# leggedrobotics/delora

Hardware: AMD Instinct MI355X
Metric: training scan-pairs/sec, KITTI 64x2048 range images (higher is better)
Workload: dtype f32; 1 GPU; KITTI-shaped 64x2048, batch=8 pairs/GPU, raw scans of ~141k points (ragged, raster order), steps rotate over 8 distinct HBM-resident batches, online normals, ResNet pose CNN (11.9M params, identity-pretrained state), Adam; BASELINE configs[1]; global_batch=8, parallelism=dp1, cnn=fp32, cnn_impl=hip trunk: fp32 MFMA, fused Winograd F(2x2,3x3) + direct implicit GEMM, channels_last=False, hip_graph=False, distinct_batches=8, priming_steps=8

## Files before the change

delora_amd/_lib.py:

```python
import ctypes
import os

_HERE = os.path.dirname(os.path.abspath(__file__))
LIB_PATH = os.path.join(_HERE, "csrc", "libdelora_hip.so")
ABI_VERSION = 10


class DeloraHipError(RuntimeError):
    pass


class SensorStruct(ctypes.Structure):
    _fields_ = [("H", ctypes.c_int32), ("W", ctypes.c_int32),
                ("hfov0", ctypes.c_double), ("hfov1", ctypes.c_double),
                ("vfov0", ctypes.c_double), ("vfov1", ctypes.c_double)]


_vp, _i32, _i64, _u32, _f32, _sz = (ctypes.c_void_p, ctypes.c_int32, ctypes.c_int64, ctypes.c_uint32,
                                    ctypes.c_float, ctypes.c_size_t)
_SP = ctypes.POINTER(SensorStruct)

SIGNATURES = {
    "dl_abi_version": (_i32, []),
    "dl_last_error": (ctypes.c_char_p, []),
    "dl_project_workspace_bytes": (_sz, [_i32, _i32, _i32, _i64, _i32]),
    "dl_project": (_i32, [_vp, _i64, _i64, _vp, _i32, _i32, _i32, _SP, _vp, _vp, _vp, _vp, _vp, _vp, _vp, _vp, _vp]),
    "dl_reproject_workspace_bytes": (_sz, [_i32, _i32, _i32]),
    "dl_reproject": (_i32, [_vp, _i64, _vp, _i64, _vp, _i64, _vp, _vp, _i32, _SP, _vp, _vp, _vp, _vp, _vp]),
    "dl_normals": (_i32, [_vp, _i64, _i32, _i32, _i32, _i32, _i32, _f32, _i32, _vp, _vp, _vp]),
    "dl_nn_workspace_bytes": (_sz, [_i32, _i32, _i32]),
    "dl_nn_correspond": (_i32, [_vp, _i64, _vp, _i64, _vp, _i64, _vp, _i64, _vp, _i32, _SP, _i32, _vp, _vp, _vp, _vp, _vp]),
    "dl_icp_loss_workspace_bytes": (_sz, [_i32, _i32, _i32]),
    "dl_icp_loss_fwd": (_i32, [_vp, _i64, _vp, _i64, _vp, _i64, _vp, _vp, _i32, _i32, _i32, _u32,
                               _vp, _vp, _vp, _vp, _vp]),
    "dl_icp_loss_partial": (_i32, [_vp, _i64, _vp, _i64, _vp, _i64, _vp, _vp, _i32, _i32, _i32, _u32, _vp, _vp]),
    "dl_icp_loss_reduce": (_i32, [_vp, _i32, _i32, _i32, _u32, _vp, _vp, _vp, _vp]),
    "dl_icp_loss_bwd": (_i32, [_vp, _vp, _i32, _vp, _vp]),
    "dl_ring_act_pool_pad_fwd": (_i32, [_vp, _i64, _i32, _i32, _i32, _vp, _vp, _vp]),
    "dl_ring_act_pool_pad_bwd": (_i32, [_vp, _vp, _vp, _i64, _i32, _i32, _i32, _vp, _vp]),
    "dl_timer_create": (_i32, [ctypes.POINTER(ctypes.c_void_p)]),
    "dl_timer_destroy": (_i32, [_vp]),
    "dl_timer_elapsed_ms": (_i32, [_vp, ctypes.POINTER(ctypes.c_float)]),
    "dl_icp_loss_partial_timed": (_i32, [_vp, _i64, _vp, _i64, _vp, _i64, _vp, _vp, _i32, _i32, _i32, _u32, _vp, _vp, _vp]),
    "dl_probe_stream_read": (_i32, [_vp, _i64, _vp, _i64, _vp, _i64, _vp, _i32, _i32, _i32, _vp, _vp]),
    "dl_nn_bruteforce": (_i32, [_vp, _i64, _i32, _vp, _i64, _i32, _vp, _vp]),
    "dl_nn_list_tree_bytes": (_sz, [_i32]),
    "dl_nn_list_query_workspace_bytes": (_sz, [_i32]),
    "dl_nn_list_build": (_i32, [_vp, _i64, _i32, _vp, _vp]),
    "dl_nn_list_query": (_i32, [_vp, _i64, _i32, _vp, _i64, _i32, _vp, _vp, _vp, _vp]),
    "dl_ring_act_pad_fwd": (_i32, [_vp, _vp, _i64, _i64, _i64, _i32, _i32, _i32, _vp, _vp]),
    "dl_ring_act_pad_bwd": (_i32, [_vp, _vp, _i64, _i32, _i32, _i32, _vp, _vp, _vp]),
    "dl_ring_act_pad_fwd_t": (_i32, [_vp, _vp, _i64, _i64, _i64, _i32, _i32, _i32, _i32, _vp, _vp]),
    "dl_ring_act_pad_bwd_t": (_i32, [_vp, _vp, _i64, _i32, _i32, _i32, _i32, _vp, _vp, _vp]),
    "dl_ring_act_pool_pad_fwd_t": (_i32, [_vp, _i64, _i32, _i32, _i32, _i32, _vp, _vp, _vp]),
    "dl_ring_act_pool_pad_bwd_t": (_i32, [_vp, _vp, _vp, _i64, _i32, _i32, _i32, _i32, _vp, _vp]),
    "dl_conv2d_nhwc_f32": (_i32, [_vp, _vp, _vp, _vp, _vp, _i32, _i32, _i32, _i32, _i32, _i32, _i32, _i32, _i32, _i32, _u32, _vp]),
    "dl_conv2d_dgrad_strided_nhwc_f32": (_i32, [_vp, _vp, _vp, _vp, _vp, _i32, _i32, _i32, _i32, _i32, _i32, _i32, _i32, _i32, _i32,
                                                _u32, _vp, _vp]),
    "dl_conv2d_wgrad_workspace_bytes": (_sz, [_i32, _i32, _i32, _i32, _i32, _i32, _i32, _i32]),
    "dl_conv2d_wgrad_nhwc_f32": (_i32, [_vp, _vp, _vp, _vp, _i32, _i32, _i32, _i32, _i32, _i32, _i32, _i32, _vp]),
    "dl_tower_conv3x3_nhwc_f32": (_i32, [_vp, _vp, _vp, _vp, _i32, _i32, _i32, _i32, _i32, _vp, _vp, _vp, _i32, _i32, _u32, _vp]),
    "dl_tower_wgrad_workspace_bytes": (_sz, [_i32, _i32, _i32, _i32, _i32]),
    "dl_tower_wgrad3x3_nhwc_f32": (_i32, [_vp, _vp, _vp, _vp, _i32, _i32, _i32, _i32, _i32, _vp, _vp, _vp]),
    "dl_wino_weights_floats": (_sz, [_i32, _i32]),
    "dl_wino_weights_f32": (_i32, [_vp, _vp, _vp, _i32, _i32, _vp]),
    "dl_wino_weights_batch_f32": (_i32, [_vp, _i32, _vp]),
    "dl_wino_conv3x3_workspace_bytes": (_sz, [_i32, _i32, _i32, _i32, _i32]),
    "dl_wino_conv3x3_nhwc_f32": (_i32, [_vp, _vp, _vp, _vp, _vp, _i32, _i32, _i32, _i32, _i32, _i32, _u32, _vp, _vp]),
    "dl_wino_wgrad_workspace_bytes": (_sz, [_i32, _i32, _i32, _i32, _i32]),
    "dl_wino_wgrad3x3_nhwc_f32": (_i32, [_vp, _vp, _vp, _vp, _i32, _i32, _i32, _i32, _i32, _vp]),
    "dl_pool3x3s12_nhwc_fwd": (_i32, [_vp, _i32, _i32, _i32, _i32, _vp, _vp, _vp]),
    "dl_pool3x3s12_nhwc_bwd": (_i32, [_vp, _vp, _vp, _i32, _i32, _i32, _i32, _i32, _vp, _vp]),
    "dl_stem_wgrad_workspace_bytes": (_sz, [_i32, _i32, _i32]),
    "dl_stem_wgrad_f32": (_i32, [_vp, _vp, _vp, _vp, _i32, _i32, _i32, _i32, _vp, _vp, _vp]),
    "dl_quat_to_T_fwd": (_i32, [_vp, _vp, _i32, ctypes.c_float, _vp, _vp]),
    "dl_quat_to_T_bwd": (_i32, [_vp, _vp, _i32, ctypes.c_float, _vp, _vp, _vp]),
    "dl_mean_hw_nhwc_f32": (_i32, [_vp, _i32, _i32, _i32, _vp, _vp]),
    "dl_conv_weights_h": (_i32, [_vp, _vp, _vp, _i32, _i32, _i32, _i32, _vp]),
    "dl_conv_weights_batch_h": (_i32, [_vp, _i32, _i32, _vp]),
    "dl_conv2d_nhwc_h": (_i32, [_vp, _vp, _vp, _vp, _vp, _i32, _i32, _i32, _i32, _i32, _i32, _i32, _i32, _i32, _i32, _i32, _u32, _vp]),
    "dl_conv2d_dgrad_strided_nhwc_h": (_i32, [_vp, _vp, _vp, _vp, _vp, _i32, _i32, _i32, _i32, _i32, _i32, _i32, _i32, _i32, _i32, _i32,
                                              _u32, _vp, _vp]),
    "dl_cast_f32_to_h": (_i32, [_vp, _vp, _i64, _i32, _vp]),
    "dl_heads_fwd": (_i32, [_vp, _vp, _i32, _i32, _i32, _i32, _i32, _vp, _vp, _vp, _vp, _vp, _vp, _vp]),
    "dl_heads_bwd_workspace_bytes": (_sz, [_i32, _i32, _i32, _i32]),
    "dl_heads_bwd": (_i32, [_vp, _vp, _i32, _i32, _i32, _i32, _i32, _vp, _vp, _vp, _vp, _vp, _vp, _vp, _vp, _vp, _vp]),
    "dl_heads_fwd_drop": (_i32, [_vp, _vp, _i32, _i32, _i32, _i32, _i32, _vp, _vp, _vp, _vp, _vp, _vp, _vp, _vp]),
    "dl_heads_bwd_drop": (_i32, [_vp, _vp, _i32, _i32, _i32, _i32, _i32, _vp, _vp, _vp, _vp, _vp, _vp, _vp, _vp, _vp, _vp, _vp]),
    "dl_heads_single_fwd": (_i32, [_vp, _vp, _i32, _i32, _i32, _i32, _i32, _i32, _i32, _i32, _vp, _vp, _vp, _vp, _vp, _vp, _vp]),
# ... 120 lines not shown
```

delora_amd/csrc/conv.hip:

```cpp
#include <type_traits>

#include "common.h"
#include "conv_geom.h"

typedef float f32x16 __attribute__((ext_vector_type(16)));
typedef float f32x4 __attribute__((ext_vector_type(4)));

__device__ __forceinline__ __amdgpu_buffer_rsrc_t cv_rsrc(const float* base, unsigned bytes) {
  return __builtin_amdgcn_make_buffer_rsrc(const_cast<float*>(base), 0, (int)bytes, 0x00020000);
}
__device__ __forceinline__ f32x4 cv_ld16(__amdgpu_buffer_rsrc_t rs, unsigned voff, unsigned soff) {
  return __builtin_bit_cast(f32x4, __builtin_amdgcn_raw_buffer_load_b128(rs, (int)voff, (int)soff, 0));
}
#define CV_ZERO_OFF 0x80000000u

#define CV_THREADS 256
#define CV_EPI_ADD 1u
#define CV_EPI_ACT 2u
#define CV_EPI_DACT 4u
#define CV_EPI_ADD_GRID 8u
#define CV_ACT_NONE 0
#define CV_ACT_TANH 1
#define CV_ACT_RELU 2

struct ConvArgs {
  const float* x;
  const float* w;
  float* y;
  const float* add;
  const float* dsrc;
  int N, H, W, C, K, Ho, Wo;
  int act;
  unsigned epi;
  int Hout, Wout;
  int wrap;
  const float* seam;
};

__device__ __forceinline__ float cv_act(float v, int act) {
  if (act == CV_ACT_TANH) return dl_tanh(v);
  if (act == CV_ACT_RELU) return v < 0.f ? 0.f : v;
  return v;
}
__device__ __forceinline__ float cv_dact(float y, int act) {
  if (act == CV_ACT_TANH) return 1.f - y * y;
  if (act == CV_ACT_RELU) return y <= 0.f ? 0.f : 1.f;
  return 1.f;
}

__device__ __forceinline__ int cv_xcd_swizzle(int id, int n) {
  const int q = n / 8, r = n % 8, xcd = id % 8, k = id / 8;
  return (xcd < r ? xcd * (q + 1) : r * (q + 1) + (xcd - r) * q) + k;
}

template <int BM, int BN, int CK, int TW, class G, bool BT, int WGN>
#ifndef CV_MINWAVES
#define CV_MINWAVES 2
#endif
__global__ __launch_bounds__(CV_THREADS, CV_MINWAVES) void k_conv_f32(ConvArgs a) {
  constexpr int TH = BM / TW;
  constexpr int SH = G::ISH, SW = G::ISW;
  constexpr int RH = (TH - 1) * SH + G::EH, RW = (TW - 1) * SW + G::EW;
  constexpr int S = CK + 4;
  constexpr int TAPS = G::NT;
  constexpr int C4 = CK / 4;
  constexpr int IN_FLOATS = RH * RW * S;
  constexpr int W_FLOATS = BT ? TAPS * CK * BN : TAPS * BN * S;
  constexpr int NI = RH * RW * C4;
  constexpr int NW = BT ? CK * TAPS * (BN / 4) : BN * TAPS * C4;
  constexpr int NI_IT = (NI + CV_THREADS - 1) / CV_THREADS, NW_IT = (NW + CV_THREADS - 1) / CV_THREADS;
  constexpr int WGM = 4 / WGN;
  constexpr int WM = BM / 32 / WGM, WN = BN / 32 / WGN;
  static_assert(BM % TW == 0 && BM % (32 * WGM) == 0 && BN % (32 * WGN) == 0 && CK % 8 == 0, "tile shape");
  static_assert(TAPS > 0, "a stride phase without taps has no launch");
  static_assert((S / 4) % 2 == 1, "pixel stride must be 4*odd floats");
  constexpr int EPW = WN * 32, ES = EPW + 4;
  constexpr int LDS_HOLD = (BM == 256 && TW == 128 && CK == 8 && BT) ? 160 * 1024 / 3 / 4 + 16 : 0;
  constexpr int LDS_USED = IN_FLOATS + W_FLOATS > 4 * 32 * ES ? IN_FLOATS + W_FLOATS : 4 * 32 * ES;
  constexpr int LDS_FLOATS = LDS_USED > LDS_HOLD ? LDS_USED : LDS_HOLD;
  __shared__ __attribute__((aligned(16))) float lds[LDS_FLOATS];
  float* in_lds = lds;
  float* w_lds = lds + IN_FLOATS;

  const int tid = threadIdx.x, lane = tid & 63, wave = tid >> 6;
  const int li = lane & 31, half = lane >> 5;
  const int wm = wave / WGN, wn = wave % WGN;
  const int KT = a.K / BN;
  const int tiles_w = (a.Wo + TW - 1) / TW, tiles_h = (a.Ho + TH - 1) / TH;
  const int ntiles = a.N * tiles_h * tiles_w * KT;
  const int t = cv_xcd_swizzle(blockIdx.x, ntiles);
  const int kt = t % KT;
  int pt = t / KT;
  const int tw_i = pt % tiles_w; pt /= tiles_w;
  const int th_i = pt % tiles_h;
  const int n = pt / tiles_h;
  const int ho0 = th_i * TH, wo0 = tw_i * TW, k0 = kt * BN;
  const int h_base = ho0 * SH + G::H0, w_base = wo0 * SW + G::W0;
  const float* xn = a.x + (size_t)n * a.H * a.W * a.C;

  const unsigned x_bytes = (unsigned)(a.H * a.W * a.C) * 4u, w_bytes = (unsigned)(a.K * a.C * G::WTAPS) * 4u;
  const __amdgpu_buffer_rsrc_t x_rs = cv_rsrc(xn, x_bytes), w_rs = cv_rsrc(a.w, w_bytes);
  const unsigned x_zero = CV_ZERO_OFF;
  unsigned in_g[NI_IT];
  int in_l[NI_IT];
#pragma unroll
  for (int it = 0; it < NI_IT; ++it) {
    const int q = min(tid + it * CV_THREADS, NI - 1);
    const int c4 = q % C4, pc = q / C4;
    const int col = pc % RW, row = pc / RW;
    const int h = h_base + row;
    int w = w_base + col;
    const bool col_in = w >= 0 && w < a.W;
    w = w < 0 ? w + a.W : w;
    w = w >= a.W ? w - a.W : w;
    in_l[it] = pc * S + c4 * 4;
    in_g[it] = (h >= 0 && h < a.H && (a.wrap ? w < a.W : col_in)) ? (unsigned)((h * a.W + w) * a.C + c4 * 4) * 4u : x_zero;
  }
  unsigned w_g[NW_IT];
  int w_l[NW_IT];
#pragma unroll
  for (int it = 0; it < NW_IT; ++it) {
    const int q = min(tid + it * CV_THREADS, NW - 1);
    if (!BT) {
      const int c4 = q % C4, t2 = q / C4;
      const int tap = t2 % TAPS, kk = t2 / TAPS;
      w_g[it] = (unsigned)(((k0 + kk) * G::WTAPS + G::wt(tap)) * a.C + c4 * 4) * 4u;
      w_l[it] = (tap * BN + kk) * S + c4 * 4;
    } else {
      const int co4 = q % (BN / 4), t2 = q / (BN / 4);
      const int tap = t2 % TAPS, kr = t2 / TAPS;
      w_g[it] = (unsigned)((kr * G::WTAPS + G::wt(tap)) * a.K + k0 + co4 * 4) * 4u;
      w_l[it] = (tap * CK + kr) * BN + co4 * 4;
    }
  }

  f32x16 acc[WM][WN];
#pragma unroll
  for (int i = 0; i < WM; ++i)
#pragma unroll
    for (int j = 0; j < WN; ++j)
#pragma unroll
      for (int r = 0; r < 16; ++r) acc[i][j][r] = 0.f;

  int a_off[WM];
#pragma unroll
  for (int mi = 0; mi < WM; ++mi) {
    const int p = (wm * WM + mi) * 32 + li;
    const int th = p / TW, tw = p % TW;
    a_off[mi] = ((th * SH) * RW + tw * SW) * S + half * 4;
  }

  f32x4 in_r[NI_IT], w_r[NW_IT];
#define CV_FETCH(C0)                                                                                                      \
  {                                                                                                                       \
    const unsigned xs_ = (unsigned)(C0) * 4u, ws_ = BT ? (unsigned)((C0) * G::WTAPS * a.K) * 4u : xs_;          \
    _Pragma("unroll") for (int it = 0; it < NI_IT; ++it) in_r[it] = cv_ld16(x_rs, in_g[it], xs_);                         \
    _Pragma("unroll") for (int it = 0; it < NW_IT; ++it) w_r[it] = cv_ld16(w_rs, w_g[it], ws_);                           \
  }
#define CV_STAGE()                                                                                                        \
  {                                                                                                                       \
    _Pragma("unroll") for (int it = 0; it < NI_IT; ++it) *reinterpret_cast<f32x4*>(in_lds + in_l[it]) = in_r[it];         \
    _Pragma("unroll") for (int it = 0; it < NW_IT; ++it) *reinterpret_cast<f32x4*>(w_lds + w_l[it]) = w_r[it];            \
  }

  CV_FETCH(0)
  CV_STAGE()
  __syncthreads();
  for (int c0 = 0; c0 < a.C; c0 += CK) {
    const bool more = c0 + CK < a.C;
    if (more) CV_FETCH(c0 + CK)
#ifdef CV_OLD_LOOP
#pragma unroll
    for (int tap = 0; tap < TAPS; ++tap) {
#pragma unroll
      for (int kq = 0; kq < CK / 8; ++kq) {
        float4 af[WM];
#pragma unroll
        for (int mi = 0; mi < WM; ++mi)
          af[mi] = *reinterpret_cast<const float4*>(in_lds + a_off[mi] + (G::dh(tap) * RW + G::dw(tap)) * S + kq * 8);
        float bf[WN][4];
#pragma unroll
        for (int ni = 0; ni < WN; ++ni) {
          const int col = (wn * WN + ni) * 32 + li;
          if (!BT) {
            const float4 v = *reinterpret_cast<const float4*>(w_lds + (tap * BN + col) * S + kq * 8 + half * 4);
            bf[ni][0] = v.x; bf[ni][1] = v.y; bf[ni][2] = v.z; bf[ni][3] = v.w;
          } else {
#pragma unroll
            for (int j = 0; j < 4; ++j) bf[ni][j] = w_lds[(tap * CK + kq * 8 + half * 4 + j) * BN + col];
          }
        }
#pragma unroll
        for (int j = 0; j < 4; ++j)
#pragma unroll
          for (int mi = 0; mi < WM; ++mi) {
            const float av = j == 0 ? af[mi].x : (j == 1 ? af[mi].y : (j == 2 ? af[mi].z : af[mi].w));
#pragma unroll
            for (int ni = 0; ni < WN; ++ni)
              acc[mi][ni] = __builtin_amdgcn_mfma_f32_32x32x2f32(av, bf[ni][j], acc[mi][ni], 0, 0, 0);
          }
      }
    }
#else
    constexpr int KQ = CK / 8, NSTEP = TAPS * KQ;
    float4 af[2][WM];
    float bf[2][WN][4];
    auto load_frags = [&](int step, int buf) {
      const int tap = step / KQ, kq = step % KQ;
#pragma unroll
      for (int mi = 0; mi < WM; ++mi)
        af[buf][mi] = *reinterpret_cast<const float4*>(in_lds + a_off[mi] + (G::dh(tap) * RW + G::dw(tap)) * S + kq * 8);
#pragma unroll
      for (int ni = 0; ni < WN; ++ni) {
        const int col = (wn * WN + ni) * 32 + li;
        if (!BT) {
          const float4 v = *reinterpret_cast<const float4*>(w_lds + (tap * BN + col) * S + kq * 8 + half * 4);
          bf[buf][ni][0] = v.x; bf[buf][ni][1] = v.y; bf[buf][ni][2] = v.z; bf[buf][ni][3] = v.w;
        } else {
#pragma unroll
          for (int j = 0; j < 4; ++j) bf[buf][ni][j] = w_lds[(tap * CK + kq * 8 + half * 4 + j) * BN + col];
        }
      }
    };
    load_frags(0, 0);
#pragma unroll
    for (int step = 0; step < NSTEP; ++step) {
      const int cur = step & 1;
      if (step + 1 < NSTEP) load_frags(step + 1, cur ^ 1);
#pragma unroll
      for (int j = 0; j < 4; ++j)
#pragma unroll
        for (int mi = 0; mi < WM; ++mi) {
          const float av = j == 0 ? af[cur][mi].x : (j == 1 ? af[cur][mi].y : (j == 2 ? af[cur][mi].z : af[cur][mi].w));
#pragma unroll
          for (int ni = 0; ni < WN; ++ni)
            acc[mi][ni] = __builtin_amdgcn_mfma_f32_32x32x2f32(av, bf[cur][ni][j], acc[mi][ni], 0, 0, 0);
        }
#ifndef CV_NO_SGB
      if (step + 1 < NSTEP) __builtin_amdgcn_sched_group_barrier(0x100, WM + (BT ? 4 * WN : WN), 0);
      __builtin_amdgcn_sched_group_barrier(0x008, 4 * WM * WN, 0);
#endif
    }
#endif
    __syncthreads();
    if (more) {
      CV_STAGE()
      __syncthreads();
    }
  }

  __syncthreads();
  float* ep = lds + wave * (32 * ES);
  const unsigned out_n = (unsigned)(n * a.Hout * a.Wout), grid_n = (unsigned)(n * a.Ho * a.Wo);
  const unsigned k_lane = (unsigned)(k0 + wn * EPW);
  const bool f_add = a.epi & CV_EPI_ADD, f_act = a.epi & CV_EPI_ACT, f_dact = a.epi & CV_EPI_DACT;
  const bool f_addg = a.epi & CV_EPI_ADD_GRID;
#pragma unroll
  for (int mi = 0; mi < WM; ++mi) {
#pragma unroll
    for (int ni = 0; ni < WN; ++ni)
#pragma unroll
      for (int r = 0; r < 16; ++r) ep[((r & 3) + 8 * (r >> 2) + 4 * half) * ES + ni * 32 + li] = acc[mi][ni][r];
#pragma unroll 2
    for (int q = lane; q < 32 * (EPW / 4); q += 64) {
      const int row = q / (EPW / 4), c4 = q % (EPW / 4);
      const int p = (wm * WM + mi) * 32 + row;
      const int th = p / TW, tw = p % TW;
      const int oh = (ho0 + th) * G::OSH + G::OPH, ow = (wo0 + tw) * G::OSW + G::OPW;
      if (ho0 + th >= a.Ho || wo0 + tw >= a.Wo || oh >= a.Hout || ow >= a.Wout) continue;
      const unsigned o = (out_n + (unsigned)(oh * a.Wout + ow)) * (unsigned)a.K + k_lane + c4 * 4;
      float4 v = *reinterpret_cast<const float4*>(ep + row * ES + c4 * 4);
      if (a.seam && (ow == 0 || ow == a.Wout - 1)) {
        const float4 t = *reinterpret_cast<const float4*>(a.seam + ((unsigned)((n * a.Hout + oh) * 2 + (ow != 0)) * (unsigned)a.K + k_lane + c4 * 4));
        v.x += t.x; v.y += t.y; v.z += t.z; v.w += t.w;
      }
      if (f_addg) {
        const float4 t = *reinterpret_cast<const float4*>(a.add + ((grid_n + (unsigned)((ho0 + th) * a.Wo + (wo0 + tw))) * (unsigned)a.K + k_lane + c4 * 4));
        v.x += t.x; v.y += t.y; v.z += t.z; v.w += t.w;
      }
      if (f_add) {
        const float4 t = *reinterpret_cast<const float4*>(a.add + o);
        v.x += t.x; v.y += t.y; v.z += t.z; v.w += t.w;
      }
      if (f_act) { v.x = cv_act(v.x, a.act); v.y = cv_act(v.y, a.act); v.z = cv_act(v.z, a.act); v.w = cv_act(v.w, a.act); }
      if (f_dact) {
        const float4 t = *reinterpret_cast<const float4*>(a.dsrc + o);
        v.x *= cv_dact(t.x, a.act); v.y *= cv_dact(t.y, a.act); v.z *= cv_dact(t.z, a.act); v.w *= cv_dact(t.w, a.act);
      }
      *reinterpret_cast<float4*>(a.y + o) = v;
    }
  }
}

#undef CV_FETCH
#undef CV_STAGE

struct WgArgs {
  const float* x;
  const float* g;
  float* part;
  int N, H, W, C, K, Ho, Wo, chunks_per_slab, nslabs;
};
template <int BMK, int BNC, int PK, int SH, int SW, int KS, bool FAST>
__device__ __forceinline__ void wgrad_f32_body(const float* __restrict__ x, const float* __restrict__ g, float* __restrict__ part, int N, int H,
                                               int W, int C, int K, int Ho, int Wo, int chunks_per_slab, int nslabs, const int blk) {
  constexpr int PAD = (KS - 1) / 2;
  constexpr int TAPS = KS * KS;
  constexpr int RW = (PK - 1) * SW + KS;
  constexpr int X_FLOATS = KS * RW * BNC, G_FLOATS = PK * BMK;
  constexpr int NX = KS * RW * (BNC / 4), NG = PK * (BMK / 4);
  constexpr int NX_IT = (NX + CV_THREADS - 1) / CV_THREADS, NG_IT = (NG + CV_THREADS - 1) / CV_THREADS;
  constexpr int TM = BMK / 32, TN = BNC / 32;
  constexpr int TILES = TM * TN;
  static_assert(TILES % 4 == 0, "tile count");
  constexpr int TPW = TILES / 4;
  __shared__ __attribute__((aligned(16))) float lds[X_FLOATS + G_FLOATS];
  float* x_lds = lds;
  float* g_lds = lds + X_FLOATS;
  const int tid = threadIdx.x, lane = tid & 63, wave = tid >> 6;
  const int li = lane & 31, half = lane >> 5;
  const int KT = K / BMK, CT = C / BNC;
  int t = blk;
// ... 373 lines not shown
  }
}

extern "C" int dl_conv2d_nhwc_f32(const float* x, const float* w, float* y, const float* add, const float* dsrc, int32_t N,
                                  int32_t H, int32_t W, int32_t C, int32_t K, int32_t ksize, int32_t stride_h,
                                  int32_t stride_w, int32_t transposed, int32_t act, uint32_t epilogue, dl_stream stream) {
  if (!x || !w || !y || N <= 0 || H <= 0 || W <= 0 || C <= 0 || K <= 0)
    return dl_fail(DL_ERR_INVALID_ARGUMENT, "dl_conv2d_nhwc_f32: bad argument");
  if (((epilogue & CV_EPI_ADD) && !add) || ((epilogue & CV_EPI_DACT) && !dsrc) || act < 0 || act > 2 || (epilogue & ~7u))
    return dl_fail(DL_ERR_INVALID_ARGUMENT, "dl_conv2d_nhwc_f32: epilogue operand missing / bad activation or flag");
  if ((stride_h != 1 && stride_h != 2) || (stride_w != 1 && stride_w != 2) || (ksize != 1 && ksize != 3))
    return dl_fail(DL_ERR_INVALID_ARGUMENT, "dl_conv2d_nhwc_f32: kernel size must be 1 or 3, strides 1 or 2 (got %d, %d, %d)", ksize, stride_h, stride_w);
  if ((size_t)N * H * W * C >= ((size_t)1 << 31) || (size_t)N * H * W * K >= ((size_t)1 << 31))
    return dl_fail(DL_ERR_UNSUPPORTED, "dl_conv2d_nhwc_f32: tensors beyond 2^31 elements are not supported (split the batch)");
  if ((size_t)H * W * C >= ((size_t)1 << 29) || (size_t)K * C * ksize * ksize >= ((size_t)1 << 29))
    return dl_fail(DL_ERR_UNSUPPORTED, "dl_conv2d_nhwc_f32: an image or the weights of 2 GiB and more are not supported");
  const int Ho = (H + stride_h - 1) / stride_h, Wo = (W + stride_w - 1) / stride_w;
  ConvArgs a{x, w, y, add, dsrc, N, H, W, C, K, Ho, Wo, act, epilogue, Ho, Wo, 1, nullptr};
  hipStream_t st = (hipStream_t)stream;
  int rc = 1;
  if (ksize == 3 && stride_h == 1 && stride_w == 1)
    rc = transposed ? dispatch_conv<GeomDgrad<3, 1, 1, 0, 0, false>, true, true>(a, st) : dispatch_conv<GeomConv<3, 1, 1>, false, true>(a, st);
  else if (transposed) return dl_fail(DL_ERR_UNSUPPORTED, "dl_conv2d_nhwc_f32: transposed weights need stride 1, 3x3 (strided layers: dl_conv2d_dgrad_strided_nhwc_f32)");
  else if (ksize == 3 && stride_h == 1 && stride_w == 2) rc = dispatch_conv<GeomConv<3, 1, 2>, false, false>(a, st);
  else if (ksize == 3 && stride_h == 2 && stride_w == 2) rc = dispatch_conv<GeomConv<3, 2, 2>, false, false>(a, st);
  else if (ksize == 1 && stride_h == 1 && stride_w == 2) rc = dispatch_conv<GeomConv<1, 1, 2>, false, false>(a, st);
  else if (ksize == 1 && stride_h == 2 && stride_w == 2) rc = dispatch_conv<GeomConv<1, 2, 2>, false, false>(a, st);
  else return dl_fail(DL_ERR_UNSUPPORTED, "dl_conv2d_nhwc_f32: kernel %d stride (%d,%d) is not built", ksize, stride_h, stride_w);
  if (rc) return dl_fail(DL_ERR_UNSUPPORTED, "dl_conv2d_nhwc_f32: shape N=%d H=%d W=%d C=%d K=%d does not tile (K %% %d, C %% 8)",
                         N, H, W, C, K, CV_BN);
  return dl_check_launch("dl_conv2d_nhwc_f32");
}

template <int KS, int SH, int SW, int PH, int PW>
static int dgrad_phase(ConvArgs a, bool first_phase, hipStream_t st) {
  using G = GeomDgrad<KS, SH, SW, PH, PW, true>;
  if (!first_phase) a.epi &= ~CV_EPI_ADD_GRID;
  if constexpr (G::NT > 0) return dispatch_conv<G, true, false>(a, st);
  return 1;
}

extern "C" int dl_conv2d_dgrad_strided_nhwc_f32(const float* g, const float* w, float* dx, const float* add_grid, const float* dsrc,
                                                int32_t N, int32_t H, int32_t W, int32_t K, int32_t C, int32_t ksize,
                                                int32_t stride_h, int32_t stride_w, int32_t dense, int32_t act,
                                                uint32_t epilogue, float* seam_ws, dl_stream stream) {
  if (!g || !w || !dx || N <= 0 || H <= 0 || W <= 0 || C <= 0 || K <= 0)
    return dl_fail(DL_ERR_INVALID_ARGUMENT, "dl_conv2d_dgrad_strided_nhwc_f32: bad argument");
  if (((epilogue & CV_EPI_ADD_GRID) && !add_grid) || ((epilogue & CV_EPI_DACT) && !dsrc) || act < 0 || act > 2 ||
      (epilogue & ~(CV_EPI_ADD_GRID | CV_EPI_DACT)))
    return dl_fail(DL_ERR_INVALID_ARGUMENT, "dl_conv2d_dgrad_strided_nhwc_f32: epilogue operand missing / unsupported flag");
  if ((stride_h != 1 && stride_h != 2) || (stride_w != 1 && stride_w != 2) || (ksize != 1 && ksize != 3))
    return dl_fail(DL_ERR_INVALID_ARGUMENT, "dl_conv2d_dgrad_strided_nhwc_f32: kernel size must be 1 or 3, strides 1 or 2 (got %d, %d, %d)", ksize, stride_h, stride_w);
  const int Ho = (H + stride_h - 1) / stride_h, Wo = (W + stride_w - 1) / stride_w;
  if ((size_t)N * H * W * C >= ((size_t)1 << 31) || (size_t)N * Ho * Wo * K >= ((size_t)1 << 31))
    return dl_fail(DL_ERR_UNSUPPORTED, "dl_conv2d_dgrad_strided_nhwc_f32: tensors beyond 2^31 elements are not supported");
  if ((size_t)Ho * Wo * K >= ((size_t)1 << 29) || (size_t)K * C * ksize * ksize >= ((size_t)1 << 29))
    return dl_fail(DL_ERR_UNSUPPORTED, "dl_conv2d_dgrad_strided_nhwc_f32: an image or the weights of 2 GiB and more are not supported");
  const bool odd_w = stride_w == 2 && (W & 1) && ksize == 3 && !dense && W >= 3;
  if (odd_w && !seam_ws)
    return dl_fail(DL_ERR_INVALID_ARGUMENT, "dl_conv2d_dgrad_strided_nhwc_f32: an odd image width (%d) needs seam_ws (N*H*2*C floats)", W);
  ConvArgs a{g, w, dx, add_grid, dsrc, N, Ho, Wo, K, C, Ho, Wo, act, epilogue, dense ? Ho : H, dense ? Wo : W, odd_w ? 0 : 1,
             odd_w ? seam_ws : nullptr};
  hipStream_t st = (hipStream_t)stream;
  if (odd_w) {
    const int row_tiles = (H + FX_ROWS - 1) / FX_ROWS;
    DL_LAUNCH_PLAIN(k_dgrad_oddw_seam, dim3(N * row_tiles, 2, (C + 63) / 64), dim3(CV_THREADS), st, g, w, seam_ws, N, Ho, Wo, K, C, H, stride_h);
// ... 208 lines not shown
```

delora_amd/csrc/conv_geom.h:

```cpp
#pragma once

template <int KS_, int SH_, int SW_>
struct GeomConv {
  static constexpr int NT = KS_ * KS_, WTAPS = KS_ * KS_, ISH = SH_, ISW = SW_;
  static constexpr int H0 = -((KS_ - 1) / 2), W0 = -((KS_ - 1) / 2), EH = KS_, EW = KS_;
  static constexpr int OSH = 1, OSW = 1, OPH = 0, OPW = 0;
  static constexpr int dh(int t) { return t / KS_; }
  static constexpr int dw(int t) { return t % KS_; }
  static constexpr int wt(int t) { return t; }
};

template <int KS_, int S_, int P_>
struct DgradAxis {
  static constexpr int PAD = (KS_ - 1) / 2;
  static constexpr bool valid(int r) { return (P_ + PAD - r) % S_ == 0; }
  static constexpr int off(int r) { return (P_ + PAD - r) / S_; }
  static constexpr int count() { int n = 0; for (int r = 0; r < KS_; ++r) n += valid(r) ? 1 : 0; return n; }
  static constexpr int tap(int i) { int n = 0; for (int r = 0; r < KS_; ++r) if (valid(r)) { if (n == i) return r; ++n; } return 0; }
  static constexpr int lo() { int m = 99; for (int r = 0; r < KS_; ++r) if (valid(r) && off(r) < m) m = off(r); return m; }
  static constexpr int hi() { int m = -99; for (int r = 0; r < KS_; ++r) if (valid(r) && off(r) > m) m = off(r); return m; }
};

template <int KS_, int SH_, int SW_, int PH_, int PW_, bool SO_>
struct GeomDgrad {
  using AH = DgradAxis<KS_, SH_, PH_>;
  using AW = DgradAxis<KS_, SW_, PW_>;
  static constexpr int NR = AH::count(), NS = AW::count();
  static constexpr int NT = NR * NS, WTAPS = KS_ * KS_, ISH = 1, ISW = 1;
  static constexpr int H0 = AH::lo(), W0 = AW::lo(), EH = AH::hi() - AH::lo() + 1, EW = AW::hi() - AW::lo() + 1;
  static constexpr int OSH = SO_ ? SH_ : 1, OSW = SO_ ? SW_ : 1, OPH = SO_ ? PH_ : 0, OPW = SO_ ? PW_ : 0;
  static constexpr int dh(int t) { return AH::off(AH::tap(t / NS)) - H0; }
  static constexpr int dw(int t) { return AW::off(AW::tap(t % NS)) - W0; }
  static constexpr int wt(int t) { return AH::tap(t / NS) * KS_ + AW::tap(t % NS); }
};
```

delora_amd/models/ring_conv.py:

```python
import ctypes
import os

import torch

from .. import _lib

ACT = {"none": 0, "tanh": 1, "relu": 2}
USE_WINOGRAD = True
EPI_ADD, EPI_ACT, EPI_DACT, EPI_ADD_GRID = 1, 2, 4, 8


def _ptr(t):
    return ctypes.c_void_p(t.data_ptr()) if t is not None else ctypes.c_void_p(0)


def _stream():
    return ctypes.c_void_p(torch.cuda.current_stream().cuda_stream)


ALLOC_SKEW = 0
_skew_state = {"i": 0}


def _empty(shape, dtype, device):
# ... 4 lines not shown
        n *= int(d)
    esz = torch.empty((), dtype=dtype).element_size()
    _skew_state["i"] = (_skew_state["i"] + 1) % 8
    off = (_skew_state["i"] * ALLOC_SKEW) // esz
    return torch.empty((n + (8 * ALLOC_SKEW) // esz,), dtype=dtype, device=device)[off:off + n].view(shape)


def weight_storage(w):
    v = w.permute(0, 2, 3, 1)
    return v if v.is_contiguous() else v.contiguous()


def grad_for(dw_krsc, w_param):
    shape, stride = (tuple(w_param.shape), tuple(w_param.stride())) if torch.is_tensor(w_param) else w_param
    g = dw_krsc.permute(0, 3, 1, 2)
    if tuple(g.stride()) != stride and shape[2] == 1 and shape[3] == 1 and stride[0] == shape[1] and stride[1] == 1:
        g = g.as_strided(shape, stride)
    return g


def out_size(n, stride):
    return -(-int(n) // int(stride))


def conv_nhwc(x, w_krsc, stride=(1, 1), act=0, epilogue=0, add=None, dsrc=None, transposed=False):
    lib = _lib.load()
    N, H, W, C = x.shape
    ks = w_krsc.shape[1]
    K = w_krsc.shape[3] if transposed else w_krsc.shape[0]
    y = _empty((N, out_size(H, stride[0]), out_size(W, stride[1]), K), torch.float32, x.device)
    _lib.check(lib.dl_conv2d_nhwc_f32(_ptr(x), _ptr(w_krsc), _ptr(y), _ptr(add), _ptr(dsrc), N, H, W, C, K, ks, stride[0],
                                      stride[1], int(transposed), int(act), int(epilogue), _stream()), "dl_conv2d_nhwc_f32")
    return y


USE_WINOGRAD_WGRAD = True


def wgrad_nhwc(x, g, ks, stride=(1, 1)):
    lib = _lib.load()
    N, H, W, C = x.shape
    K = g.shape[3]
    dw = torch.empty((K, ks, ks, C), dtype=torch.float32, device=x.device)
    if USE_WINOGRAD_WGRAD and ks == 3 and tuple(stride) == (1, 1) and C >= 128:
        nbytes = lib.dl_wino_wgrad_workspace_bytes(N, H, W, C, K)
        if nbytes:
            ws = torch.empty((nbytes // 4,), dtype=torch.float32, device=x.device)
            _lib.check(lib.dl_wino_wgrad3x3_nhwc_f32(_ptr(x), _ptr(g), _ptr(dw), _ptr(ws), N, H, W, C, K, _stream()),
                       "dl_wino_wgrad3x3_nhwc_f32")
            return dw
    ws = torch.empty((lib.dl_conv2d_wgrad_workspace_bytes(N, H, W, C, K, ks, stride[0], stride[1]) // 4,), dtype=torch.float32,
                     device=x.device)
    _lib.check(lib.dl_conv2d_wgrad_nhwc_f32(_ptr(x), _ptr(g), _ptr(dw), _ptr(ws), N, H, W, C, K, ks, stride[0], stride[1],
                                            _stream()), "dl_conv2d_wgrad_nhwc_f32")
    return dw


def _wgrad_layer_table(part):
    arr = (_lib.WgradLayer * len(part))()
    dws = []
    for j, (x, g, ks, stride) in enumerate(part):
        N, H, W, C = x.shape
        K = g.shape[3]
        dw = torch.empty((K, ks, ks, C), dtype=torch.float32, device=x.device)
        dws.append(dw)
        arr[j].x, arr[j].g, arr[j].dw = x.data_ptr(), g.data_ptr(), dw.data_ptr()
# ... 501 lines not shown
        return [(b, b + 1) for b in range(nb)]
    if mode == "layer":
        cuts = [b for b in range(1, nb) if blocks[b][3] and blocks[b][0] >= 128]
        edges = [0] + cuts + [nb]
        return [(edges[i], edges[i + 1]) for i in range(len(edges) - 1)]
    return [(0, nb)]


class RingSegment(torch.autograd.Function):

    @staticmethod
    def forward(ctx, x0, act, blocks, first, last, *weights):
        saved, x, wi = [x0], x0, 0
        ubwd = []
        need_bwd = any(ctx.needs_input_grad)
        plan, (N, H, W) = [], x0.shape[:3]
        for (cin, cout, stride, has_ds) in blocks:
            use1 = USE_WINOGRAD and stride == (1, 1) and wino_ok(H, W, cin, cout)
            H, W = out_size(H, stride[0]), out_size(W, stride[1])
            use2 = USE_WINOGRAD and wino_ok(H, W, cout, cout)
            plan.append((use1, use2))
        wlist, wj = [], 0
        for (cin, cout, stride, has_ds), (use1, use2) in zip(blocks, plan):
            if use1:
                wlist.append(weights[wj])
            if use2:
                wlist.append(weights[wj + 1])
            wj += 3 if has_ds else 2
        us = iter(wino_weights_batch(wlist, want_bwd=need_bwd))
        for (cin, cout, stride, has_ds), (use1, use2) in zip(blocks, plan):
            w1p, w2p = weights[wi], weights[wi + 1]
            wd = weight_storage(weights[wi + 2]) if has_ds else None
            wi += 3 if has_ds else 2
            if use1:
                uf, ub1 = next(us)
                y1 = wino_conv(x, uf, cout, act=act, epilogue=EPI_ACT)
            else:
                ub1 = None
                y1 = conv_nhwc(x, weight_storage(w1p), stride=stride, act=act, epilogue=EPI_ACT)
            shortcut = conv_nhwc(x, wd, stride=stride) if has_ds else x
            if use2:
                uf, ub2 = next(us)
                y2 = wino_conv(y1, uf, cout, act=act, epilogue=EPI_ADD | EPI_ACT, add=shortcut)
            else:
                ub2 = None
                y2 = conv_nhwc(y1, weight_storage(w2p), act=act, epilogue=EPI_ADD | EPI_ACT, add=shortcut)
            ubwd += [ub1, ub2]
            saved += [y1, y2]
            x = y2
        dsrc0 = first if torch.is_tensor(first) else None
        ctx.act, ctx.blocks, ctx.first, ctx.last = act, blocks, dsrc0 is None and bool(first), last
        ctx.ubwd_mask = tuple(u is not None for u in ubwd)
        ctx.has_dsrc0 = dsrc0 is not None
        ctx.save_for_backward(*saved, *weights, *[u for u in ubwd if u is not None], *([dsrc0] if dsrc0 is not None else []))
        return x

    @staticmethod
    def backward(ctx, dy):
        act, blocks = ctx.act, ctx.blocks
        nb = len(blocks)
        saved = ctx.saved_tensors
        dsrc0 = None
        if ctx.has_dsrc0:
            saved, dsrc0 = saved[:-1], saved[-1]
        nu = sum(ctx.ubwd_mask)
        acts, weights = saved[:1 + 2 * nb], saved[1 + 2 * nb:len(saved) - nu]
        u_it = iter(saved[len(saved) - nu:])
        ubwd = [next(u_it) if has else None for has in ctx.ubwd_mask]
        grads = [None] * len(weights)
        g2 = dy.contiguous()
        if ctx.last:
            y_last = acts[-1]
            if act == ACT["tanh"]:
# ... 268 lines not shown
```

include/delora_hip.h:

```cpp
#ifndef DELORA_HIP_H
#define DELORA_HIP_H

#include <stddef.h>
#include <stdint.h>

#ifdef __cplusplus
extern "C" {
#endif

#define DL_ABI_VERSION 10

typedef void* dl_stream;

typedef enum {
  DL_OK = 0,
  DL_ERR_INVALID_ARGUMENT = -1,
  DL_ERR_LAUNCH = -2,
  DL_ERR_UNSUPPORTED = -3
} dl_status;

typedef struct {
  int32_t H;
  int32_t W;
  double hfov0, hfov1;
// ... 68 lines not shown
int dl_nn_list_build(const float* tgt, int64_t mt_cs, int32_t Mt, void* tree, dl_stream stream);
int dl_nn_list_query(const float* src, int64_t ms_cs, int32_t Ms, const float* tgt, int64_t mt_cs, int32_t Mt,
                     const void* tree, int32_t* nn, void* workspace, dl_stream stream);

int dl_ring_act_pad_fwd(const float* x, const float* res, int64_t res_pitch, int64_t res_off, int64_t rows,
                        int32_t W, int32_t pad, int32_t act, float* out, dl_stream stream);
int dl_ring_act_pad_bwd(const float* grad_out, const float* y, int64_t rows, int32_t W, int32_t pad, int32_t act,
                        float* grad_x, float* grad_res_padded, dl_stream stream);

int dl_ring_act_pool_pad_fwd(const float* x, int64_t planes, int32_t H, int32_t W, int32_t act, float* out, int8_t* win,
                             dl_stream stream);
int dl_ring_act_pool_pad_bwd(const float* grad_out, const float* y, const int8_t* win, int64_t planes, int32_t H,
                             int32_t W, int32_t act, float* grad_x, dl_stream stream);

#define DL_DTYPE_F32  0
#define DL_DTYPE_F16  1
#define DL_DTYPE_BF16 2

int dl_ring_act_pad_fwd_t(const void* x, const void* res, int64_t res_pitch, int64_t res_off, int64_t rows, int32_t W, int32_t pad,
                          int32_t act, int32_t dtype, void* out, dl_stream stream);
int dl_ring_act_pad_bwd_t(const void* grad_out, const void* y, int64_t rows, int32_t W, int32_t pad, int32_t act, int32_t dtype,
                          void* grad_x, void* grad_res_padded, dl_stream stream);
int dl_ring_act_pool_pad_fwd_t(const void* x, int64_t planes, int32_t H, int32_t W, int32_t act, int32_t dtype, void* out, int8_t* win,
                               dl_stream stream);
int dl_ring_act_pool_pad_bwd_t(const void* grad_out, const void* y, const int8_t* win, int64_t planes, int32_t H, int32_t W,
                               int32_t act, int32_t dtype, void* grad_x, dl_stream stream);

#define DL_CONV_ADD  1u
#define DL_CONV_ACT  2u
#define DL_CONV_DACT 4u
int dl_conv2d_nhwc_f32(const float* x, const float* w, float* y, const float* add, const float* dsrc, int32_t N,
                       int32_t H, int32_t W, int32_t C, int32_t K, int32_t ksize, int32_t stride_h, int32_t stride_w,
                       int32_t transposed, int32_t act, uint32_t epilogue, dl_stream stream);

#define DL_CONV_ADD_GRID 8u
int dl_conv2d_dgrad_strided_nhwc_f32(const float* g, const float* w, float* dx, const float* add_grid, const float* dsrc,
                                     int32_t N, int32_t H, int32_t W, int32_t K, int32_t C, int32_t ksize,
                                     int32_t stride_h, int32_t stride_w, int32_t dense, int32_t act, uint32_t epilogue,
                                     float* seam_ws, dl_stream stream);

size_t dl_conv2d_wgrad_workspace_bytes(int32_t N, int32_t H, int32_t W, int32_t C, int32_t K, int32_t ksize,
                                       int32_t stride_h, int32_t stride_w);
int dl_conv2d_wgrad_nhwc_f32(const float* x, const float* g, float* dw, void* workspace, int32_t N, int32_t H, int32_t W,
                             int32_t C, int32_t K, int32_t ksize, int32_t stride_h, int32_t stride_w, dl_stream stream);

int dl_tower_conv3x3_nhwc_f32(const float* x, const float* w, float* y, const float* dsrc, int32_t N, int32_t H, int32_t W,
                              int32_t C, int32_t K, const int32_t* x_view, const int32_t* y_view, const int32_t* dsrc_view,
                              int32_t transposed, int32_t act, uint32_t epilogue, dl_stream stream);
size_t dl_tower_wgrad_workspace_bytes(int32_t N, int32_t H, int32_t W, int32_t C, int32_t K);
int dl_tower_wgrad3x3_nhwc_f32(const float* x, const float* g, float* dw, void* workspace, int32_t N, int32_t H, int32_t W,
                               int32_t C, int32_t K, const int32_t* x_view, const int32_t* g_view, dl_stream stream);

size_t dl_wino_weights_floats(int32_t K, int32_t C);
int dl_wino_weights_f32(const float* w, float* u_fwd, float* u_bwd, int32_t K, int32_t C, dl_stream stream);
#define DL_WINO_BATCH 16
typedef struct {
  const float* w;
  float* u_fwd;
  float* u_bwd;
  int32_t K, C;
} dl_wino_layer;
int dl_wino_weights_batch_f32(const dl_wino_layer* layers, int32_t n, dl_stream stream);
size_t dl_wino_conv3x3_workspace_bytes(int32_t N, int32_t H, int32_t W, int32_t C, int32_t K);
int dl_wino_conv3x3_nhwc_f32(const float* x, const float* u, float* y, const float* add, const float* dsrc, int32_t N,
                             int32_t H, int32_t W, int32_t C, int32_t K, int32_t act, uint32_t epilogue, void* workspace,
                             dl_stream stream);
// ... 131 lines not shown
```

Before: 677.2 scan-pairs/s.

## Fuse downsample 1x1 shortcut conv into strided 3x3 forward conv kernel

Result: no change. 679.0 scan-pairs/s (median of 6 runs) (+0.3%).

```diff
diff --git a/delora_amd/_lib.py b/delora_amd/_lib.py
--- a/delora_amd/_lib.py
+++ b/delora_amd/_lib.py
@@ -55,6 +55,7 @@
     "dl_ring_act_pool_pad_fwd_t": (_i32, [_vp, _i64, _i32, _i32, _i32, _i32, _vp, _vp, _vp]),
     "dl_ring_act_pool_pad_bwd_t": (_i32, [_vp, _vp, _vp, _i64, _i32, _i32, _i32, _i32, _vp, _vp]),
     "dl_conv2d_nhwc_f32": (_i32, [_vp, _vp, _vp, _vp, _vp, _i32, _i32, _i32, _i32, _i32, _i32, _i32, _i32, _i32, _i32, _u32, _vp]),
+    "dl_conv2d_shortcut_nhwc_f32": (_i32, [_vp, _vp, _vp, _vp, _vp, _i32, _i32, _i32, _i32, _i32, _i32, _i32, _i32, _u32, _vp]),
     "dl_conv2d_dgrad_strided_nhwc_f32": (_i32, [_vp, _vp, _vp, _vp, _vp, _i32, _i32, _i32, _i32, _i32, _i32, _i32, _i32, _i32, _i32,
                                                 _u32, _vp, _vp]),
     "dl_conv2d_wgrad_workspace_bytes": (_sz, [_i32, _i32, _i32, _i32, _i32, _i32, _i32, _i32]),
diff --git a/delora_amd/csrc/conv.hip b/delora_amd/csrc/conv.hip
--- a/delora_amd/csrc/conv.hip
+++ b/delora_amd/csrc/conv.hip
@@ -35,6 +35,8 @@
   int Hout, Wout;
   int wrap;
   const float* seam;
+  const float* wd;
+  float* yd;
 };
 
 __device__ __forceinline__ float cv_act(float v, int act) {
@@ -52,12 +54,16 @@
   const int q = n / 8, r = n % 8, xcd = id % 8, k = id / 8;
   return (xcd < r ? xcd * (q + 1) : r * (q + 1) + (xcd - r) * q) + k;
 }
+
+template <class G> struct cv_geom_ds { static constexpr bool value = false; };
+template <int SH_, int SW_> struct cv_geom_ds<GeomConvDs<3, SH_, SW_>> { static constexpr bool value = true; };
 
 template <int BM, int BN, int CK, int TW, class G, bool BT, int WGN>
 #ifndef CV_MINWAVES
 #define CV_MINWAVES 2
 #endif
 __global__ __launch_bounds__(CV_THREADS, CV_MINWAVES) void k_conv_f32(ConvArgs a) {
+  constexpr bool DS = cv_geom_ds<G>::value;
   constexpr int TH = BM / TW;
   constexpr int SH = G::ISH, SW = G::ISW;
   constexpr int RH = (TH - 1) * SH + G::EH, RW = (TW - 1) * SW + G::EW;
@@ -65,10 +71,14 @@
   constexpr int TAPS = G::NT;
   constexpr int C4 = CK / 4;
   constexpr int IN_FLOATS = RH * RW * S;
-  constexpr int W_FLOATS = BT ? TAPS * CK * BN : TAPS * BN * S;
+  static_assert(!DS || (!BT && G::WTAPS == 9 && TAPS == 9), "the fused shortcut rides on the forward pass of a 3x3 layer");
+  constexpr int CEN = 4;
+  constexpr int W_FLOATS = BT ? TAPS * CK * BN : (TAPS + (DS ? 1 : 0)) * BN * S;
   constexpr int NI = RH * RW * C4;
   constexpr int NW = BT ? CK * TAPS * (BN / 4) : BN * TAPS * C4;
+  constexpr int ND = BN * C4;
   constexpr int NI_IT = (NI + CV_THREADS - 1) / CV_THREADS, NW_IT = (NW + CV_THREADS - 1) / CV_THREADS;
+  constexpr int ND_IT = DS ? (ND + CV_THREADS - 1) / CV_THREADS : 1;
   constexpr int WGM = 4 / WGN;
   constexpr int WM = BM / 32 / WGM, WN = BN / 32 / WGN;
   static_assert(BM % TW == 0 && BM % (32 * WGM) == 0 && BN % (32 * WGN) == 0 && CK % 8 == 0, "tile shape");
@@ -133,6 +143,15 @@
       w_l[it] = (tap * CK + kr) * BN + co4 * 4;
     }
   }
+  unsigned wd_g[ND_IT];
+  if constexpr (DS) {
+#pragma unroll
+    for (int it = 0; it < ND_IT; ++it) {
+      const int q = min(tid + it * CV_THREADS, ND - 1);
+      const int c4 = q % C4, kk = q / C4;
+      wd_g[it] = (unsigned)((k0 + kk) * a.C + c4 * 4) * 4u;
+    }
+  }
 
   f32x16 acc[WM][WN];
 #pragma unroll
@@ -141,6 +160,15 @@
     for (int j = 0; j < WN; ++j)
 #pragma unroll
       for (int r = 0; r < 16; ++r) acc[i][j][r] = 0.f;
+  f32x16 acc_d[DS ? WM : 1][DS ? WN : 1];
+  if constexpr (DS) {
+#pragma unroll
+    for (int i = 0; i < WM; ++i)
+#pragma unroll
+      for (int j = 0; j < WN; ++j)
+#pragma unroll
+        for (int r = 0; r < 16; ++r) acc_d[i][j][r] = 0.f;
+  }
 
   int a_off[WM];
 #pragma unroll
@@ -150,17 +178,27 @@
     a_off[mi] = ((th * SH) * RW + tw * SW) * S + half * 4;
   }
 
-  f32x4 in_r[NI_IT], w_r[NW_IT];
+  f32x4 in_r[NI_IT], w_r[NW_IT], wd_r[ND_IT];
 #define CV_FETCH(C0)                                                                                                      \
   {                                                                                                                       \
     const unsigned xs_ = (unsigned)(C0) * 4u, ws_ = BT ? (unsigned)((C0) * G::WTAPS * a.K) * 4u : xs_;          \
     _Pragma("unroll") for (int it = 0; it < NI_IT; ++it) in_r[it] = cv_ld16(x_rs, in_g[it], xs_);                         \
     _Pragma("unroll") for (int it = 0; it < NW_IT; ++it) w_r[it] = cv_ld16(w_rs, w_g[it], ws_);                           \
+    if constexpr (DS) {                                                   \
+      const __amdgpu_buffer_rsrc_t wd_rs_ = cv_rsrc(a.wd, (unsigned)(a.K * a.C) * 4u);                                    \
+      _Pragma("unroll") for (int it = 0; it < ND_IT; ++it) wd_r[it] = cv_ld16(wd_rs_, wd_g[it], xs_);                     \
+    }                                                                                                                     \
   }
 #define CV_STAGE()                                                                                                        \
   {                                                                                                                       \
     _Pragma("unroll") for (int it = 0; it < NI_IT; ++it) *reinterpret_cast<f32x4*>(in_lds + in_l[it]) = in_r[it];         \
     _Pragma("unroll") for (int it = 0; it < NW_IT; ++it) *reinterpret_cast<f32x4*>(w_lds + w_l[it]) = w_r[it];            \
+    if constexpr (DS) {          \
+      _Pragma("unroll") for (int it = 0; it < ND_IT; ++it) {                                                              \
+        const int q_ = min(tid + it * CV_THREADS, ND - 1);                                                                \
+        *reinterpret_cast<f32x4*>(w_lds + (TAPS * BN + q_ / C4) * S + (q_ % C4) * 4) = wd_r[it];                          \
+      }                                                                                                                   \
+    }                                                                                                                     \
   }
 
   CV_FETCH(0)
@@ -202,14 +240,15 @@
       }
     }
 #else
-    constexpr int KQ = CK / 8, NSTEP = TAPS * KQ;
+    constexpr int KQ = CK / 8, NSTEP = (TAPS + (DS ? 1 : 0)) * KQ;
     float4 af[2][WM];
     float bf[2][WN][4];
     auto load_frags = [&](int step, int buf) {
       const int tap = step / KQ, kq = step % KQ;
+      const int atap = DS && tap == TAPS ? CEN : tap;
 #pragma unroll
       for (int mi = 0; mi < WM; ++mi)
-        af[buf][mi] = *reinterpret_cast<const float4*>(in_lds + a_off[mi] + (G::dh(tap) * RW + G::dw(tap)) * S + kq * 8);
+        af[buf][mi] = *reinterpret_cast<const float4*>(in_lds + a_off[mi] + (G::dh(atap) * RW + G::dw(atap)) * S + kq * 8);
 #pragma unroll
       for (int ni = 0; ni < WN; ++ni) {
         const int col = (wn * WN + ni) * 32 + li;
@@ -233,8 +272,10 @@
         for (int mi = 0; mi < WM; ++mi) {
           const float av = j == 0 ? af[cur][mi].x : (j == 1 ? af[cur][mi].y : (j == 2 ? af[cur][mi].z : af[cur][mi].w));
 #pragma unroll
-          for (int ni = 0; ni < WN; ++ni)
-            acc[mi][ni] = __builtin_amdgcn_mfma_f32_32x32x2f32(av, bf[cur][ni][j], acc[mi][ni], 0, 0, 0);
+          for (int ni = 0; ni < WN; ++ni) {
+            if (DS && step / KQ == TAPS) acc_d[mi][ni] = __builtin_amdgcn_mfma_f32_32x32x2f32(av, bf[cur][ni][j], acc_d[mi][ni], 0, 0, 0);
+            else acc[mi][ni] = __builtin_amdgcn_mfma_f32_32x32x2f32(av, bf[cur][ni][j], acc[mi][ni], 0, 0, 0);
+          }
         }
 #ifndef CV_NO_SGB
       if (step + 1 < NSTEP) __builtin_amdgcn_sched_group_barrier(0x100, WM + (BT ? 4 * WN : WN), 0);
@@ -288,6 +329,24 @@
         v.x *= cv_dact(t.x, a.act); v.y *= cv_dact(t.y, a.act); v.z *= cv_dact(t.z, a.act); v.w *= cv_dact(t.w, a.act);
       }
       *reinterpret_cast<float4*>(a.y + o) = v;
+    }
+  }
+  if constexpr (DS) {
+#pragma unroll
+    for (int mi = 0; mi < WM; ++mi) {
+#pragma unroll
+      for (int ni = 0; ni < WN; ++ni)
+#pragma unroll
+        for (int r = 0; r < 16; ++r) ep[((r & 3) + 8 * (r >> 2) + 4 * half) * ES + ni * 32 + li] = acc_d[mi][ni][r];
+#pragma unroll 2
+      for (int q = lane; q < 32 * (EPW / 4); q += 64) {
+        const int row = q / (EPW / 4), c4 = q % (EPW / 4);
+        const int p = (wm * WM + mi) * 32 + row;
+        const int th = p / TW, tw = p % TW;
+        if (ho0 + th >= a.Ho || wo0 + tw >= a.Wo) continue;
+        const unsigned o = (grid_n + (unsigned)((ho0 + th) * a.Wo + (wo0 + tw))) * (unsigned)a.K + k_lane + c4 * 4;
+        *reinterpret_cast<float4*>(a.yd + o) = *reinterpret_cast<const float4*>(ep + row * ES + c4 * 4);
+      }
     }
   }
 }
@@ -727,6 +786,52 @@
   return dl_check_launch("dl_conv2d_nhwc_f32");
 }
 
+template <int BM, int TW, class G, int WGN>
+static int launch_conv_ds(const ConvArgs& a, hipStream_t st) {
+  constexpr int TH = BM / TW, BN = 64, CK = 8;
+  const int ntiles = a.N * ((a.Ho + TH - 1) / TH) * ((a.Wo + TW - 1) / TW) * (a.K / BN);
+  const double px_ = (double)a.N * a.Ho * a.Wo;
+  const DlProfTag tag{"k_conv_f32", "fwd+ds", a.N, a.H, a.W, a.C, a.K, 3, G::ISH, G::ISW, 2.0 * px_ * a.K * a.C * 10,
+                      4.0 * ((double)a.N * a.H * a.W * a.C + 2 * px_ * a.K + 10.0 * a.K * a.C)};
+  DL_LAUNCH(tag, (k_conv_f32<BM, BN, CK, TW, G, false, WGN>), dim3(ntiles), dim3(CV_THREADS), st, a);
+  return 0;
+}
+template <class G>
+static int dispatch_conv_ds(const ConvArgs& a, hipStream_t st) {
+  if constexpr (G::ISH == 1 && G::ISW == 2) {
+    if (a.Wo % 128 == 0 && a.Ho % 2 == 0) return launch_conv_ds<256, 128, G, 1>(a, st);
+  }
+  switch (cv_pick_tw(a.Ho, a.Wo, 128, 16)) {
+    case 128: return launch_conv_ds<128, 128, G, CV_WGN>(a, st);
+    case 64: return launch_conv_ds<128, 64, G, CV_WGN>(a, st);
+    case 32: return launch_conv_ds<128, 32, G, CV_WGN>(a, st);
+    default: return launch_conv_ds<128, 16, G, CV_WGN>(a, st);
+  }
+}
+
+extern "C" int dl_conv2d_shortcut_nhwc_f32(const float* x, const float* w, const float* w_ds, float* y, float* y_ds, int32_t N, int32_t H,
+                                           int32_t W, int32_t C, int32_t K, int32_t stride_h, int32_t stride_w, int32_t act,
+                                           uint32_t epilogue, dl_stream stream) {
+  if (!x || !w || !w_ds || !y || !y_ds || N <= 0 || H <= 0 || W <= 0 || C <= 0 || K <= 0)
+    return dl_fail(DL_ERR_INVALID_ARGUMENT, "dl_conv2d_shortcut_nhwc_f32: bad argument");
+  if (act < 0 || act > 2 || (epilogue & ~CV_EPI_ACT))
+    return dl_fail(DL_ERR_INVALID_ARGUMENT, "dl_conv2d_shortcut_nhwc_f32: bad activation or flag (the epilogue is 0 or DL_CONV_ACT)");
+  if (!((stride_h == 1 || stride_h == 2) && stride_w == 2))
+    return dl_fail(DL_ERR_UNSUPPORTED, "dl_conv2d_shortcut_nhwc_f32: stride (%d,%d) is not built (the down-sampling blocks' (1,2) and (2,2) are)", stride_h, stride_w);
+  if ((size_t)N * H * W * C >= ((size_t)1 << 31) || (size_t)N * H * W * K >= ((size_t)1 << 31))
+    return dl_fail(DL_ERR_UNSUPPORTED, "dl_conv2d_shortcut_nhwc_f32: tensors beyond 2^31 elements are not supported (split the batch)");
+  if ((size_t)H * W * C >= ((size_t)1 << 29) || (size_t)K * C * 9 >= ((size_t)1 << 29))
+    return dl_fail(DL_ERR_UNSUPPORTED, "dl_conv2d_shortcut_nhwc_f32: an image or the weights of 2 GiB and more are not supported");
+  if (K % 64 || C % 8 || C > 256 || (W & 1))
+    return dl_fail(DL_ERR_UNSUPPORTED, "dl_conv2d_shortcut_nhwc_f32: shape N=%d H=%d W=%d C=%d K=%d is not fused (K %% 64, C %% 8, C <= 256, W even)", N, H, W, C, K);
+  const int Ho = (H + stride_h - 1) / stride_h, Wo = (W + stride_w - 1) / stride_w;
+  ConvArgs a{x, w, y, nullptr, nullptr, N, H, W, C, K, Ho, Wo, act, epilogue, Ho, Wo, 1, nullptr, w_ds, y_ds};
+  hipStream_t st = (hipStream_t)stream;
+  const int rc = stride_h == 1 ? dispatch_conv_ds<GeomConvDs<3, 1, 2>>(a, st) : dispatch_conv_ds<GeomConvDs<3, 2, 2>>(a, st);
+  if (rc) return dl_fail(DL_ERR_UNSUPPORTED, "dl_conv2d_shortcut_nhwc_f32: shape N=%d H=%d W=%d C=%d K=%d does not tile", N, H, W, C, K);
+  return dl_check_launch("dl_conv2d_shortcut_nhwc_f32");
+}
+
 template <int KS, int SH, int SW, int PH, int PW>
 static int dgrad_phase(ConvArgs a, bool first_phase, hipStream_t st) {
   using G = GeomDgrad<KS, SH, SW, PH, PW, true>;
diff --git a/delora_amd/csrc/conv_geom.h b/delora_amd/csrc/conv_geom.h
--- a/delora_amd/csrc/conv_geom.h
+++ b/delora_amd/csrc/conv_geom.h
@@ -9,6 +9,9 @@
   static constexpr int dw(int t) { return t % KS_; }
   static constexpr int wt(int t) { return t; }
 };
+
+template <int KS_, int SH_, int SW_>
+struct GeomConvDs : GeomConv<KS_, SH_, SW_> {};
 
 template <int KS_, int S_, int P_>
 struct DgradAxis {
diff --git a/delora_amd/models/ring_conv.py b/delora_amd/models/ring_conv.py
--- a/delora_amd/models/ring_conv.py
+++ b/delora_amd/models/ring_conv.py
@@ -60,6 +60,30 @@
     _lib.check(lib.dl_conv2d_nhwc_f32(_ptr(x), _ptr(w_krsc), _ptr(y), _ptr(add), _ptr(dsrc), N, H, W, C, K, ks, stride[0],
                                       stride[1], int(transposed), int(act), int(epilogue), _stream()), "dl_conv2d_nhwc_f32")
     return y
+
+
+FUSE_SHORTCUT = True
+
+
+def shortcut_fusable(x_shape, cout, stride):
+    N, H, W, C = (int(v) for v in x_shape)
+    if tuple(stride) not in ((1, 2), (2, 2)) or min(N, H, W, C, cout) < 1:
+        return False
+    if C % 8 or C > 256 or cout % 64 or W % 2:
+        return False
+    return N * H * W * max(C, cout) < (1 << 31) and H * W * C < (1 << 29) and 9 * C * cout < (1 << 29)
+
+
+def conv_shortcut_nhwc(x, w_krsc, wd_k11c, stride, act=0, epilogue=0):
+    lib = _lib.load()
+    N, H, W, C = x.shape
+    K = w_krsc.shape[0]
+    Ho, Wo = out_size(H, stride[0]), out_size(W, stride[1])
+    y = _empty((N, Ho, Wo, K), torch.float32, x.device)
+    yd = _empty((N, Ho, Wo, K), torch.float32, x.device)
+    _lib.check(lib.dl_conv2d_shortcut_nhwc_f32(_ptr(x), _ptr(w_krsc), _ptr(wd_k11c), _ptr(y), _ptr(yd), N, H, W, C, K, stride[0], stride[1],
+                                               int(act), int(epilogue), _stream()), "dl_conv2d_shortcut_nhwc_f32")
+    return y, yd
 
 
 USE_WINOGRAD_WGRAD = True
@@ -627,13 +651,18 @@
             w1p, w2p = weights[wi], weights[wi + 1]
             wd = weight_storage(weights[wi + 2]) if has_ds else None
             wi += 3 if has_ds else 2
+            fused = has_ds and not use1 and FUSE_SHORTCUT and shortcut_fusable(x.shape, cout, stride)
             if use1:
                 uf, ub1 = next(us)
                 y1 = wino_conv(x, uf, cout, act=act, epilogue=EPI_ACT)
+            elif fused:
+                ub1 = None
+                y1, shortcut = conv_shortcut_nhwc(x, weight_storage(w1p), wd, stride, act=act, epilogue=EPI_ACT)
             else:
                 ub1 = None
                 y1 = conv_nhwc(x, weight_storage(w1p), stride=stride, act=act, epilogue=EPI_ACT)
-            shortcut = conv_nhwc(x, wd, stride=stride) if has_ds else x
+            if not fused:
+                shortcut = conv_nhwc(x, wd, stride=stride) if has_ds else x
             if use2:
                 uf, ub2 = next(us)
                 y2 = wino_conv(y1, uf, cout, act=act, epilogue=EPI_ADD | EPI_ACT, add=shortcut)
diff --git a/include/delora_hip.h b/include/delora_hip.h
--- a/include/delora_hip.h
+++ b/include/delora_hip.h
@@ -124,6 +124,10 @@
 int dl_conv2d_nhwc_f32(const float* x, const float* w, float* y, const float* add, const float* dsrc, int32_t N,
                        int32_t H, int32_t W, int32_t C, int32_t K, int32_t ksize, int32_t stride_h, int32_t stride_w,
                        int32_t transposed, int32_t act, uint32_t epilogue, dl_stream stream);
+
+int dl_conv2d_shortcut_nhwc_f32(const float* x, const float* w, const float* w_ds, float* y, float* y_ds, int32_t N, int32_t H,
+                                int32_t W, int32_t C, int32_t K, int32_t stride_h, int32_t stride_w, int32_t act, uint32_t epilogue,
+                                dl_stream stream);
 
 #define DL_CONV_ADD_GRID 8u
 int dl_conv2d_dgrad_strided_nhwc_f32(const float* g, const float* w, float* dx, const float* add_grid, const float* dsrc,
```
